# TheDatumOrg/VAQ

Hardware: AMD Instinct MI355X
Metric: queries/sec (ADC search, recall@100 reported alongside) (higher is better)
Workload: dtype f32; 1 GPU; sift1m-shaped d128 m8x256 nq10k k100; rows=1000000, rows_per_gpu=1000000, queries_per_gpu=10000, k=100, code_bytes=8, codes=encoded, method=HEAP/EA (exhaustive)

## Files before the change

### vaq_amd/csrc/vaq_kernels.h

```cpp
#ifndef VAQ_KERNELS_H_
#define VAQ_KERNELS_H_

#include <hip/hip_runtime.h>
#include <stdint.h>

#include "refine_owner.h"

namespace vaq {

struct SubDesc {
  int ncent;
  int bits;
  int bit_off;
  int lut_off;
  int cent_off;
  int word;
  int shift;
  int pad;
};

enum Layout { LAYOUT_BYTES = 0, LAYOUT_BITS = 1 };
enum EarlyAbandon { EA_NONE = 0, EA_QUEUE = 1, EA_INPLACE = 2 };

constexpr int TILE_ROWS = 64;
// ... 19 lines not shown
  int n_buckets;
  int bucket_shift;
  int bucket_t;
  int n_hot;
  unsigned long long *stats;
  int no_skip;
  const int *first_sub;
  const float *lut;
  int lut_floats;
  int lds_subs;
  int lut_lds_entries;
  int nq;
  int k;
  int kp;
  int ccap;
  int qcap;
  int q_cw_words;
  int nwaves;
  int ea;
  unsigned *g_thr;
  int qb;
  int n_slices;
  int64_t slice_rows;
  int64_t slice_stride;
  int share_thr;
  const int *slice_order;
  const int *qorder;
  int seq;
  int32_t *final_labels;
  float *final_dist;
  int64_t id_base;
  int *part_cnt;
  int bf_carry;
  int bf_pool;
  int defer_units, defer_mode, defer_cap;
  unsigned *defer_count;
  struct DeferRec *defer_list;
  unsigned *bm_done;
  int bf;
  int ti;
  const int *ti_order;
  const float *ti_qcc;
  const int *ti_nvisit;
  const float *ti_xcc;
  int ti_rowcap;
  int ti_cap;
  int sqrt_out;
  float *part_d;
  int *part_id;
};

hipError_t launch_project(const float *X, int64_t n, int D, const float *E, float *out,
                          hipStream_t st, int checked = 0);
hipError_t launch_lut_build(const float *qproj, int nq, int D, int M, int L,
                            const SubDesc *sub, const float *cent_t, int lut_floats, int max_ncent,
                            float *lut, hipStream_t st, int min_ncent = 1);
hipError_t launch_lut_expand(const float *lut_packed, int nq, int M, const SubDesc *sub,
                             int lut_floats, int ksub, float *lut_ref, hipStream_t st);
hipError_t launch_encode(const float *Xp, int64_t n, int D, int M, int L, const SubDesc *sub,
                         const float *cent, uint16_t *codes, hipStream_t st);
hipError_t lut_fit_columns(const float *d_Xp, int64_t n, int D, const int *bits, float *d_cent_out, float *d_q_out,
                           int *d_bad, float *phase_ms, hipStream_t st);
hipError_t launch_lut_encode(const float *Xp, int64_t n, int D, const SubDesc *h_sub, const SubDesc *d_sub,
                             const float *d_pm, const float *d_cent, uint16_t *codes, int n_cu, hipStream_t st);
hipError_t launch_refine(const float *Q, int nq, int D, const float *dataset, const float *rows,
                         const int32_t *labels_in, int R, int k, int32_t *labels, float *dist,
                         hipStream_t st);
struct RowsRef {
  const void *p;
  int elem;
};
inline RowsRef rows_at(RowsRef r, size_t elems) {
  return RowsRef{static_cast<const char *>(r.p) + elems * (size_t)r.elem, r.elem};
}
size_t refine_rows_max_dim();
hipError_t lut_fit_columns(RowsRef d_Xp, int64_t n, int D, const int *bits, float *d_cent_out, float *d_q_out,
                           int *d_bad, float *phase_ms, hipStream_t st);
hipError_t launch_project(RowsRef X, int64_t n, int D, const float *E, float *out, hipStream_t st, int checked = 0);
hipError_t launch_refine_rows(const float *Q, int nq, int D, RowsRef rows, int64_t N, int64_t id_base,
                              const int32_t *labels_in, int R, int k, int exact, int32_t *labels, float *dist,
                              hipStream_t st);
hipError_t launch_refine_dist(const float *Q, int nq, int D, RowsRef rows, int64_t n, int64_t lo_label,
                              const int32_t *labels_in, int R, float *plane, hipStream_t st);
hipError_t launch_refine_select(const int32_t *labels_in, int nq, const float *planes, size_t plane_stride,
                                const RefineBounds &bounds, int R, int k, int exact, int32_t *labels, float *dist,
                                hipStream_t st);
hipError_t launch_widen_rows_u8(const uint8_t *src, int64_t elems, float *dst, hipStream_t st);
constexpr int XS_TILE = 256;
constexpr int XS_MAX_QG = 1024;
constexpr int XS_MAX_K1 = 1025;
struct XsParams {
  int nq, D;
  int64_t N, id_base;
  int k, cap;
  int S, G, qg;
  int64_t split_rows;
  float *buf_d;
  int *buf_id;
  float *part_d;
  int *part_id;
};
int exhaust_list_cap(int k);
size_t exhaust_register_max_dim();
int exhaust_blocks_per_cu(int D, int elem);
hipError_t launch_exhaust_select(const XsParams &p, const float *Q, RowsRef rows, hipStream_t st);
hipError_t launch_exhaust_replay(const float *Q, int nq, int D, RowsRef rows, int64_t N, int64_t id_base, int k,
                                 const int *list, const unsigned *count, int32_t *labels, float *dist, hipStream_t st);
hipError_t launch_exhaust_replay_link(const float *Q, int nq, int D, RowsRef rows, int64_t N, int64_t id_base, int k,
                                      const int *list, const unsigned *count, const float *hin_v, const int *hin_i,
                                      float *hout_v, int *hout_i, int finish, int32_t *labels, float *dist,
                                      hipStream_t st);
hipError_t launch_exhaust_scatter(int nq, int k, const int *list, const unsigned *count, const float *src_v,
                                  const int *src_i, int32_t *labels, float *dist, hipStream_t st);
int64_t packed_words(int64_t rows, int M, int layout, int W);
hipError_t launch_pack_codes(const uint16_t *codes_u16, int64_t row_begin, int64_t row_end,
                             int64_t out_row_end, int M, int layout, int W, const SubDesc *sub,
                             const uint32_t *perm, uint32_t *out, hipStream_t st);
hipError_t sort_by_first_code(const uint16_t *d_codes, int64_t n, int M, int bits0, int shift, int bits1,
                              int t, uint32_t *d_perm, int *d_bucket_start, hipStream_t st, int fine = 0,
                              int *d_sub_start = nullptr);
hipError_t launch_merge_rows(const uint32_t *old_codes, const uint32_t *old_perm, const int *old_start,
                             const uint32_t *new_codes, const uint32_t *new_perm, const int *new_start, int K0,
                             int64_t n_old, int64_t n_total, int M, int layout, int W, uint32_t *out_codes,
                             uint32_t *out_perm, hipStream_t st);
hipError_t launch_slice_order(const float *lut, int lut_floats, int nq, int qb, const int *bstart,
                              int n_buckets, int bucket_shift, int64_t slice_rows, int n_slices,
                              int64_t n_rows, int *order, hipStream_t st);
hipError_t launch_cost_order(const float *lut, int lut_floats, int nq, int n0, int shift, unsigned long long *keys,
                             int *order, hipStream_t st);
hipError_t launch_query_order(const float *lut, int lut_floats, int nq, int n0, int off1, int n1, int *order,
                              hipStream_t st);
void scan_geometry(int layout, int M, int k, int ea, int *kp, int *ccap, int *qcap);
size_t scan_lds_bytes(int layout, int M, int lut_floats, int qb, int k, int ea, int nwaves,
                      int n_buckets, int bucket_shift, int bucket_t);
int scan_wg_step_rows(int layout, int M);
hipError_t launch_scan(const ScanParams &p, int *grid_out, hipStream_t st);
bool scan_bf_supported(int layout, int M, int qb, int ea, int n_buckets, int seq);
size_t scan_bf_lds_bytes(int layout, int M, int lut_entries, int pool, int nwaves, int n_buckets, int bf_carry);
void scan_bf_pool_range(int k, int *lo, int *hi);
size_t merge_scratch_elems(int n_lists, int nq, int k);
hipError_t launch_defer_merge(const unsigned *defer_count, int defer_cap, const DeferRec *defer_list, int n_lists, int k,
                              const float *part_d, const int *part_id, const int *part_cnt, int64_t id_base,
                              int32_t *labels, float *dist, hipStream_t st);
hipError_t launch_merge(const float *part_d, const int *part_id, const int *part_cnt, int n_lists,
                        int64_t list_stride, int64_t query_stride, int nq, int k,
                        int64_t id_base, int in_final, int32_t *labels, float *dist,
                        unsigned *thr_out, float *scratch_d, int *scratch_id, hipStream_t st);

constexpr int BM_HIST_BINS = 64;
constexpr int BM_XCDS = 8;
struct BmParams {
  const uint32_t *codes;
  const uint32_t *perm;
  const int *bucket_start;
  int n_buckets, bucket_t;
  const int *sub_start;
  int M;
  const float *lut;
  int lut_floats;
  int nq, k, qb;
  int nwaves;
  unsigned *g_thr;
  unsigned long long *thr64;
  int init64;
  unsigned *done_key;
  unsigned *done_next;
  unsigned *fresh;
  int limit;
  int retry;
  unsigned *mask;
  int *cnt;
  int *qoff;
  int *fill;
  int *qlist;
  unsigned short *qkey;
  int *border;
  int *ioff;
  unsigned *tickets;
  int cap;
  float *cand_d;
  int *cand_id;
  unsigned *cand_cnt;
// ... 96 lines not shown
```

### vaq_amd/csrc/vaq_kernels.hip

```cpp
#include "vaq_scan.h"
#include "vaq_scan_bf.h"
#include "vaqhip_dev.h"

#include <cstring>
#include <rocprim/device/device_radix_sort.hpp>

#include <float.h>
#include <limits.h>

namespace vaq {
template <typename T>
__global__ void project_kernel(const T *__restrict__ X, int D,
                               const float *__restrict__ E, float *__restrict__ out, int checked) {
  extern __shared__ float xs[];
  __shared__ int bad;
  const int64_t r = blockIdx.x;
  if (threadIdx.x == 0) bad = 0;
  for (int j = threadIdx.x; j < D; j += blockDim.x) xs[j] = (float)X[r * D + j];
  __syncthreads();
  if (!E) {
    for (int j = threadIdx.x; j < D; j += blockDim.x)
      if (!(fabsf(xs[j]) <= FLT_MAX)) bad = 1;
    __syncthreads();
    const bool zero = checked && bad;
// ... 125 lines not shown
                                 float *__restrict__ lut, int only_small) {
  extern __shared__ float qs[];
  const int q = blockIdx.x, s = blockIdx.y;
  const SubDesc sd = sub[s];
  if ((int)(blockIdx.z * blockDim.x) >= sd.ncent) return;
  if (only_small && sd.ncent >= 8) return;
  for (int j = threadIdx.x; j < L; j += blockDim.x) qs[j] = qproj[(size_t)q * D + (size_t)s * L + j];
  __syncthreads();
  float *out = lut + (size_t)q * lut_floats + sd.lut_off;
  const float *cs = cent_t + sd.cent_off;
  const int K = sd.ncent;
#define Y(j) cs[(size_t)(j) * K + c]
  for (int c = blockIdx.z * blockDim.x + threadIdx.x; c < K; c += gridDim.z * blockDim.x) {
    float r;
    if (K >= 8) {
      float acc = 0.0f;
      for (int j = 0; j < L; j++) {
        float diff = qs[j] - Y(j);
        acc = __builtin_fmaf(diff, diff, acc);
      }
      r = acc;
    } else if (L == 1) {
      r = sqdiff(qs[0], Y(0));
    } else if (L == 2) {
      r = sqdiff(qs[0], Y(0)) + sqdiff(qs[1], Y(1));
    } else if (L == 4) {
      r = (sqdiff(qs[0], Y(0)) + sqdiff(qs[1], Y(1))) + (sqdiff(qs[2], Y(2)) + sqdiff(qs[3], Y(3)));
    } else if (L == 8) {
      float a0 = sqdiff(qs[0], Y(0)) + sqdiff(qs[4], Y(4));
      float a1 = sqdiff(qs[1], Y(1)) + sqdiff(qs[5], Y(5));
      float a2 = sqdiff(qs[2], Y(2)) + sqdiff(qs[6], Y(6));
      float a3 = sqdiff(qs[3], Y(3)) + sqdiff(qs[7], Y(7));
      r = (a0 + a1) + (a2 + a3);
    } else if (L == 12) {
      float a0 = (sqdiff(qs[0], Y(0)) + sqdiff(qs[4], Y(4))) + sqdiff(qs[8], Y(8));
      float a1 = (sqdiff(qs[1], Y(1)) + sqdiff(qs[5], Y(5))) + sqdiff(qs[9], Y(9));
      float a2 = (sqdiff(qs[2], Y(2)) + sqdiff(qs[6], Y(6))) + sqdiff(qs[10], Y(10));
      float a3 = (sqdiff(qs[3], Y(3)) + sqdiff(qs[7], Y(7))) + sqdiff(qs[11], Y(11));
      r = (a0 + a1) + (a2 + a3);
    } else {
      float res = 0.0f;
      for (int j = 0; j < L; j++) {
        float t = qs[j] - Y(j);
        res += t * t;
      }
      r = res;
    }
    out[c] = r;
  }
#undef Y
}

constexpr int LUT_QT = 8;
__global__ __launch_bounds__(256) void lut_build_batch_kernel(const float *__restrict__ qproj, int nq, int D, int L,
                                                              const SubDesc *__restrict__ sub,
                                                              const float *__restrict__ cent_t, int lut_floats,
                                                              float *__restrict__ lut) {
  extern __shared__ float qs[];
  const int q0 = blockIdx.x * LUT_QT, s = blockIdx.y;
  const SubDesc sd = sub[s];
  const int K = sd.ncent;
  if (K < 8) return;
  for (int i = threadIdx.x; i < LUT_QT * L; i += blockDim.x) {
    const int qt = i / L, j = i - qt * L;
    qs[i] = q0 + qt < nq ? qproj[(size_t)(q0 + qt) * D + (size_t)s * L + j] : 0.0f;
  }
  __syncthreads();
  const float *cs = cent_t + sd.cent_off;
  for (int c = threadIdx.x; c < K; c += blockDim.x) {
    float acc[LUT_QT];
#pragma unroll
    for (int qt = 0; qt < LUT_QT; qt++) acc[qt] = 0.0f;
    for (int j = 0; j < L; j++) {
      const float y = cs[(size_t)j * K + c];
#pragma unroll
      for (int qt = 0; qt < LUT_QT; qt++) {
        const float diff = qs[qt * L + j] - y;
        acc[qt] = __builtin_fmaf(diff, diff, acc[qt]);
      }
    }
#pragma unroll
    for (int qt = 0; qt < LUT_QT; qt++)
      if (q0 + qt < nq) lut[(size_t)(q0 + qt) * lut_floats + sd.lut_off + c] = acc[qt];
  }
}

hipError_t launch_lut_build(const float *qproj, int nq, int D, int M, int L, const SubDesc *sub,
                            const float *cent_t, int lut_floats, int max_ncent, float *lut,
                            hipStream_t st, int min_ncent) {
  if (nq == 0) return hipSuccess;
  (void)max_ncent;
  if (nq >= 2 * LUT_QT && max_ncent >= 8) {
    hipLaunchKernelGGL(lut_build_batch_kernel, dim3((nq + LUT_QT - 1) / LUT_QT, M), dim3(256),
                       LUT_QT * L * sizeof(float), st, qproj, nq, D, L, sub, cent_t, lut_floats, lut);
    hipError_t e = hipGetLastError();
    if (e != hipSuccess || min_ncent >= 8) return e;
    hipLaunchKernelGGL(lut_build_kernel, dim3(nq, M, 1), dim3(64), L * sizeof(float), st, qproj, D, L, sub, cent_t,
                       lut_floats, lut, 1);
    return hipGetLastError();
  }
  hipLaunchKernelGGL(lut_build_kernel, dim3(nq, M, 1), dim3(256), L * sizeof(float), st, qproj, D, L,
                     sub, cent_t, lut_floats, lut, 0);
  return hipGetLastError();
}

__global__ void lut_expand_kernel(const float *__restrict__ lp, int M,
                                  const SubDesc *__restrict__ sub, int lut_floats, int ksub,
                                  float *__restrict__ lr) {
  const int q = blockIdx.x, s = blockIdx.y;
  const SubDesc sd = sub[s];
  for (int c = threadIdx.x; c < ksub; c += blockDim.x)
    lr[((size_t)q * M + s) * ksub + c] =
        c < sd.ncent ? lp[(size_t)q * lut_floats + sd.lut_off + c] : 0.0f;
}

hipError_t launch_lut_expand(const float *lut_packed, int nq, int M, const SubDesc *sub,
                             int lut_floats, int ksub, float *lut_ref, hipStream_t st) {
  if (nq == 0) return hipSuccess;
  hipLaunchKernelGGL(lut_expand_kernel, dim3(nq, M), dim3(256), 0, st, lut_packed, M, sub,
                     lut_floats, ksub, lut_ref);
  return hipGetLastError();
}

__global__ void pack_codes_kernel(const uint16_t *__restrict__ in, int64_t row_begin,
                                  int64_t row_end, int M, int layout, int W,
                                  const SubDesc *__restrict__ sub, const uint32_t *__restrict__ perm,
                                  uint32_t *__restrict__ out, int64_t t_begin, int64_t t_end) {
  const int64_t t = t_begin + (int64_t)blockIdx.x * blockDim.x + threadIdx.x;
  if (t >= t_end) return;
  uint32_t v = 0;
  if (layout == LAYOUT_BYTES) {
    const int wpr = M / 4;
    const int64_t r = t / wpr;
    const int w = (int)(t - r * wpr);
    if (r >= row_begin && r < row_end) {
      const uint16_t *c = in + ((perm ? (int64_t)perm[r] : r) - row_begin) * M + w * 4;
      v = (uint32_t)(c[0] & 0xff) | ((uint32_t)(c[1] & 0xff) << 8) |
          ((uint32_t)(c[2] & 0xff) << 16) | ((uint32_t)(c[3] & 0xff) << 24);
    }
  } else {
    const int64_t tile = t / ((int64_t)TILE_ROWS * W);
    const int rem = (int)(t - tile * TILE_ROWS * W);
    const int w = rem / TILE_ROWS;
    const int64_t r = tile * TILE_ROWS + (rem % TILE_ROWS);
    if (r >= row_begin && r < row_end) {
      const int64_t src = (perm ? (int64_t)perm[r] : r) - row_begin;
      for (int s = 0; s < M; s++) {
// ... 278 lines not shown
  for (int q = wave; q < P; q += nwaves) {
    unsigned long long key = ~0ull;
    if (q < nq) {
      const float *l = lut + (size_t)q * lut_floats;
      unsigned a[2];
#pragma unroll
      for (int t = 0; t < 2; t++) {
        const int off = t == 0 ? 0 : off1, n = t == 0 ? n0 : n1;
        unsigned long long best = ~0ull;
        for (int e = lane; e < n; e += 64) {
          const float x = l[off + e];
          const unsigned long long c = ((unsigned long long)(x == x ? float_to_bits(x) : 0xffffffffu) << 32) | (unsigned)e;
          best = c < best ? c : best;
        }
#pragma unroll
        for (int o = 32; o > 0; o >>= 1) {
          const unsigned long long x = __shfl_xor(best, o);
          best = x < best ? x : best;
        }
        a[t] = (unsigned)(best & 0xffffu);
      }
      key = ((unsigned long long)((a[0] << 16) | a[1]) << 32) | (unsigned)q;
    }
    if (lane == 0) qk[q] = key;
  }
  __syncthreads();
  for (int size = 2; size <= P; size <<= 1)
    for (int stride = size >> 1; stride > 0; stride >>= 1) {
      for (int t = tid; t < (P >> 1); t += QORDER_THREADS) {
        const int i = 2 * t - (t & (stride - 1));
        const int j = i + stride;
        const unsigned long long x = qk[i], y = qk[j];
        if ((x > y) == ((i & size) == 0)) { qk[i] = y; qk[j] = x; }
      }
      __syncthreads();
    }
  for (int i = tid; i < nq; i += QORDER_THREADS) order[i] = (int)(qk[i] & 0xffffffffu);
}

hipError_t launch_query_order(const float *lut, int lut_floats, int nq, int n0, int off1, int n1, int *order,
                              hipStream_t st) {
  if (nq <= 0 || nq > QORDER_MAX) return hipErrorInvalidValue;
  int P = 2;
  while (P < nq) P <<= 1;
  const size_t lds = (size_t)P * sizeof(unsigned long long);
  hipError_t e = hipFuncSetAttribute(reinterpret_cast<const void *>(query_order_kernel),
                                     hipFuncAttributeMaxDynamicSharedMemorySize, (int)lds);
  if (e != hipSuccess) return e;
  hipLaunchKernelGGL(query_order_kernel, dim3(1), dim3(QORDER_THREADS), lds, st, lut, lut_floats, nq, n0, off1, n1, order);
  return hipGetLastError();
}

template <int NREG>
__global__ __launch_bounds__(256) void query_cost_kernel(const float *__restrict__ lut, int lut_floats, int nq, int n0,
                                                         int shift, unsigned long long *__restrict__ keys) {
  const int lane = threadIdx.x & 63;
  const int q = blockIdx.x * 4 + (threadIdx.x >> 6);
  if (q >= nq) return;
  const float *l = lut + (size_t)q * lut_floats;
  const int nb_all = n0 >> shift;
  const int stride = nb_all > 64 * NREG ? nb_all / (64 * NREG) : 1;
  const int nb = nb_all / stride;
  unsigned v[NREG];
  unsigned vmin = 0xffffffffu, vmax = 0u;
#pragma unroll
  for (int i = 0; i < NREG; i++) {
    const int b = i * 64 + lane;
    unsigned m = 0xffffffffu;
    if (b < nb) {
      const int g = (16 >> shift) > 0 ? (16 >> shift) : 1;
      const int bb = (b / g) * g * stride + (b % g);
      for (int c = bb << shift; c < ((bb + 1) << shift); c++) {
        const float x = l[c];
        const unsigned xb = x == x ? float_to_bits(x) : 0xffffffffu;
        m = xb < m ? xb : m;
      }
    }
    v[i] = m;
    vmin = m < vmin ? m : vmin;
    vmax = (m != 0xffffffffu && m > vmax) ? m : vmax;
  }
#pragma unroll
  for (int o = 32; o > 0; o >>= 1) {
    const unsigned x = (unsigned)__shfl_xor((int)vmin, o), y = (unsigned)__shfl_xor((int)vmax, o);
    vmin = x < vmin ? x : vmin;
    vmax = y > vmax ? y : vmax;
  }
  int J = 16 / stride;
  J = J < 2 ? 2 : J;
  J = nb < J ? nb : J;
  unsigned lo = vmin, hi = vmax;
  if (lo > hi) lo = hi;
  while (lo < hi) {
    const unsigned mid = lo + ((hi - lo) >> 1);
    int c = 0;
#pragma unroll
    for (int i = 0; i < NREG; i++) c += __popcll(__ballot(v[i] <= mid));
    if (c >= J) hi = mid;
    else lo = mid + 1u;
  }
  float part = 0.0f;
  int below = 0;
#pragma unroll
  for (int i = 0; i < NREG; i++) {
    const bool lt = v[i] < lo;
    part += lt ? bits_to_float(v[i]) : 0.0f;
    below += __popcll(__ballot(lt));
  }
#pragma unroll
  for (int o = 32; o > 0; o >>= 1) part += __shfl_xor(part, o);
  const float v0 = bits_to_float(vmin < 0x7f800000u ? vmin : 0x7f800000u);
  const float spread = (part + (float)(J - below) * bits_to_float(lo)) - (float)J * v0;
  const unsigned kb = (spread == spread && spread >= 0.0f) ? float_to_bits(spread) : (spread < 0.0f ? 0u : 0x7f800000u);
  if (lane == 0) keys[q] = ((unsigned long long)kb << 32) | (unsigned)q;
}

constexpr int COST_CLASSES = 4096;
__global__ __launch_bounds__(QORDER_THREADS) void cost_sort_kernel(const unsigned long long *__restrict__ keys, int nq,
                                                                   int *__restrict__ order) {
  __shared__ unsigned hist[COST_CLASSES];
  __shared__ unsigned wave_tot[QORDER_THREADS / 64];
  const int tid = threadIdx.x, lane = tid & 63, wave = tid >> 6;
  for (int i = tid; i < COST_CLASSES; i += QORDER_THREADS) hist[i] = 0u;
  __syncthreads();
  for (int i = tid; i < nq; i += QORDER_THREADS) atomicAdd(&hist[(unsigned)(keys[i] >> 51) & (COST_CLASSES - 1)], 1u);
  __syncthreads();
  constexpr int PER = COST_CLASSES / QORDER_THREADS;
  unsigned c[PER], sum = 0u;
#pragma unroll
  for (int j = 0; j < PER; j++) {
    c[j] = hist[tid * PER + j];
    sum += c[j];
  }
  unsigned inc = sum;
#pragma unroll
  for (int o = 1; o < 64; o <<= 1) {
    const unsigned x = (unsigned)__shfl_up((int)inc, o);
    if (lane >= o) inc += x;
  }
  if (lane == 63) wave_tot[wave] = inc;
  __syncthreads();
  unsigned base = inc - sum;
  for (int w = 0; w < wave; w++) base += wave_tot[w];
#pragma unroll
  for (int j = 0; j < PER; j++) {
    hist[tid * PER + j] = base;
    base += c[j];
  }
  __syncthreads();
  for (int i = tid; i < nq; i += QORDER_THREADS) {
    const unsigned long long kq = keys[i];
    const unsigned pos = atomicAdd(&hist[(unsigned)(kq >> 51) & (COST_CLASSES - 1)], 1u);
    order[pos] = (int)(kq & 0xffffffffu);
  }
}

hipError_t launch_cost_order(const float *lut, int lut_floats, int nq, int n0, int shift, unsigned long long *keys,
                             int *order, hipStream_t st) {
  if (nq <= 0 || nq > QORDER_MAX || (n0 >> shift) > 1024 || (n0 >> shift) < 1) return hipErrorInvalidValue;
  hipLaunchKernelGGL(query_cost_kernel<4>, dim3((nq + 3) / 4), dim3(256), 0, st, lut, lut_floats, nq, n0, shift, keys);
  hipError_t e = hipGetLastError();
  if (e != hipSuccess) return e;
  hipLaunchKernelGGL(cost_sort_kernel, dim3(1), dim3(QORDER_THREADS), 0, st, keys, nq, order);
  return hipGetLastError();
}

static int rows_per_item(int layout, int M) { return (layout == LAYOUT_BYTES && M < 16) ? 16 / M : 1; }

int scan_wg_step_rows(int layout, int M) { return SCAN_MAX_THREADS * rows_per_item(layout, M); }

static int queue_code_words(int layout, int M, int ea) {
  return (layout == LAYOUT_BYTES && M <= 16 && ea == EA_QUEUE) ? M / 4 - 1 : 0;
}

void scan_geometry(int layout, int M, int k, int ea, int *kp, int *ccap, int *qcap) {
  int p2 = 1;
  while (p2 < k) p2 <<= 1;
  *kp = p2;
  *ccap = VAQ_CCAP;
  *qcap = ea == EA_QUEUE ? 128 : 0;
}

size_t scan_lds_bytes(int layout, int M, int lut_floats, int qb, int k, int ea, int nwaves,
                      int n_buckets, int bucket_shift, int bucket_t) {
  int kp, ccap, qcap;
  scan_geometry(layout, M, k, ea, &kp, &ccap, &qcap);
  size_t lut = (size_t)(layout == LAYOUT_BYTES ? M * 256 : lut_floats) * 4 * qb;
  lut = (lut + 15) & ~(size_t)15;
  const size_t sb = ((size_t)SEL_HDR_WORDS * 4 + (size_t)(kp + ccap) * 8 + 15) & ~(size_t)15;
  const size_t lbb = (bucket_shift > 0 || bucket_t > 0) ? (((size_t)n_buckets * 4 * qb + 15) & ~(size_t)15) : 0;
  return lut + (size_t)qb * sb + lbb + hot_bytes(n_buckets) +
         (size_t)nwaves * qcap * 4 * (1 + qb + queue_code_words(layout, M, ea));
}

size_t scan_ti_lds_bytes(int n_clusters) { return ti_lds_bytes(n_clusters); }

hipError_t launch_scan(const ScanParams &p_in, int *grid_out, hipStream_t st) {
  ScanParams p = p_in;
  p.q_cw_words = queue_code_words(p.layout, p.M, p.ea);
  const int nqb = (p.nq + p.qb - 1) / p.qb;
  const int total = nqb * p.n_slices;
  const int grid = ((total + 7) / 8) * 8;
  if (grid_out) *grid_out = grid;
  if (total == 0) return hipSuccess;
  if (p.bf) return launch_scan_bf(p, grid, st);
  size_t lds = scan_lds_bytes(p.layout, p.M, p.lut_lds_entries, p.qb, p.k, p.ea, p.nwaves, p.n_buckets,
                              p.bucket_shift, p.bucket_t);
  if (p.bucket_t < 0 || p.bucket_t > GMIN_MAX_BITS || (p.bucket_t > 0 && p.bucket_shift != 0))
    return hipErrorInvalidValue;
  if (p.ti) {
    if (p.qb != 1 || p.ea != EA_QUEUE || p.bucket_shift != 0 || p.bucket_t != 0 || p.n_hot != 0 || !p.sqrt_out)
      return hipErrorInvalidValue;
    if (p.ti_cap < 1 || p.ti_cap > p.n_buckets) return hipErrorInvalidValue;
    lds += ti_lds_bytes(p.ti_cap);
  } else if (p.sqrt_out) {
    return hipErrorInvalidValue;
  }
// ... 286 lines not shown
```

### vaq_amd/csrc/vaqhip_search.cpp

```cpp
#include "vaqhip_index.h"

using namespace vaqhost;

int vaqhost::check_search_args(const vaqhip_index *ix, const float *d_queries, int nq, int k, const int32_t *d_labels,
                               const float *d_dist, const char *method_err) {
  if (ix->N < 0) return fail(VAQHIP_ESTATE, "search before codes were set");
  if (ix->staged.open)
    return fail(VAQHIP_ESTATE, "a staged search is open on this index: call vaqhip_search_finish_device first");
  if (method_err) return fail(VAQHIP_ESTATE, "%s", method_err);
  if (nq < 0 || k <= 0) return fail(VAQHIP_EINVAL, "nq=%d k=%d", nq, k);
  if (k > VAQHIP_MAX_K) return fail(VAQHIP_EUNSUPPORTED, "k=%d > %d", k, VAQHIP_MAX_K);
  if (nq > 0 && (!d_queries || !d_labels || !d_dist)) return fail(VAQHIP_EINVAL, "null pointer");
  return VAQHIP_OK;
}

namespace {
int report_bm_debug(vaqhip_index *ix, const vaq::BmParams &bp, const int *limits, int r, const BmRoundInfo &bi,
                    hipStream_t st) {
  const int chunk = bi.chunk, n = bi.n;
  std::vector<unsigned> hq((size_t)3 * chunk);
  std::vector<int> hcnt((size_t)ix->n_buckets);
  HIP_TRY(hipStreamSynchronize(st));
  HIP_TRY(hipMemcpy(hq.data(), ix->w_bm_query.p, hq.size() * 4, hipMemcpyDeviceToHost));
  HIP_TRY(hipMemcpy(hcnt.data(), bp.cnt, hcnt.size() * 4, hipMemcpyDeviceToHost));
// ... 197 lines not shown
               "buckets tested %.1f visited %.1f | cycles total %.0f setup %.0f stepload-wait %.0f admit %.0f "
               "(fold %.0f lock-wait %.0f) drain %.0f | best-first: bootstrap %.0f round prep %.0f final (wave 0) %.0f setup up to the tables %.0f\n",
               h[0] / w, h[1] / w, h[2] / w, h[3] / w, h[4] / w, h[5] / w, h[9] / w, h[10] / w, h[6] / w, h[11] / w,
               h[12] / w, h[7] / w, h[13] / w, h[14] / w, h[8] / w, h[15] / w, h[16] / w, (double)h[17] / grid, h[18] / w);
  return VAQHIP_OK;
}
#endif

int group_queries(vaqhip_index *ix, const Plan &pl, int n, vaq::ScanParams &sp, hipStream_t st) {
  if (!(ix->ti_T == 0 && pl.qb > 1 && ix->M > 1 && n <= 16384 && !pl.ordered &&
        (ix->opt_group == 2 ||
         (ix->opt_group == 1 && n >= 4 * pl.qb && (double)ix->N * ((ix->total_bits + 7) / 8) > 256e6))))
    return VAQHIP_OK;
  HIP_TRY(ix->w_qorder.ensure((size_t)n * sizeof(int)));
  HIP_TRY(vaq::launch_query_order(ix->w_lut.as<float>(), ix->lut_floats, n, ix->sub[0].ncent, ix->sub[1].lut_off,
                                  ix->sub[1].ncent, ix->w_qorder.as<int>(), st));
  sp.qorder = ix->w_qorder.as<int>();
  return VAQHIP_OK;
}

int scan_chunk_ti(vaqhip_index *ix, const Plan &pl, const float *qp, int n, int k, vaq::ScanParams sp, int32_t *labels,
                  float *dist, hipEvent_t *ev, int *grid, hipStream_t st) {
  const int T = ix->ti_T;
  const int max_visit = ix->ti_visit < 1.0f ? (int)((float)T * ix->ti_visit) : T;
  HIP_TRY(vaq::launch_ti_plan(qp, n, ix->D, ix->ti_seg * ix->L, ix->d_ti_clusters_t.as<float>(), T,
                              ix->d_bstart.as<int>(), max_visit, k, ix->w_ti_order.as<int>(),
                              ix->w_ti_qcc.as<float>(), ix->w_ti_nvisit.as<int>(), st));
  if (ev) HIP_TRY(hipEventRecord(ev[3], st));
  sp.ti = 1;
  sp.ti_order = ix->w_ti_order.as<int>();
  sp.ti_qcc = ix->w_ti_qcc.as<float>();
  sp.ti_nvisit = ix->w_ti_nvisit.as<int>();
  sp.ti_xcc = ix->d_ti_xcc.as<float>();
  sp.ti_rowcap = (ix->methods & VAQHIP_METHOD_EA) ? 0x7fffffff : k;
  sp.ti_cap = pl.ti_cap;
  sp.sqrt_out = 1;
  sp.n_slices = pl.n_slices;
  sp.share_thr = pl.n_slices > 1;
  const bool direct = pl.n_slices == 1 && ix->N > 0;
  if (direct) {
    sp.final_labels = labels;
    sp.final_dist = dist;
  }
  if (ix->N > 0) HIP_TRY(vaq::launch_scan(sp, grid, st));
  if (ev) HIP_TRY(hipEventRecord(ev[4], st));
  if (!direct)
    HIP_TRY(vaq::launch_merge(sp.part_d, sp.part_id, nullptr, ix->N > 0 ? pl.n_slices : 0, k,
                              (int64_t)pl.n_slices * k, n, k, ix->id_base, 0, labels, dist, nullptr,
                              ix->w_ms_d.as<float>(), ix->w_ms_id.as<int>(), st));
  if (ev) HIP_TRY(hipEventRecord(ev[5], st));
  return VAQHIP_OK;
}

int seed_prepass(vaqhip_index *ix, const Plan &pl, int n, int k, vaq::ScanParams &sp, hipStream_t st) {
  if (ix->N > 0 && pl.seed_slices > 0) {
    sp.n_slices = pl.seed_slices;
    sp.slice_rows = pl.seed_rows;
    sp.slice_stride = pl.seed_stride;
    sp.share_thr = 1;
    sp.nwaves = 4;
    HIP_TRY(vaq::launch_scan(sp, nullptr, st));
    sp.nwaves = pl.nwaves;
    HIP_TRY(vaq::launch_merge(sp.part_d, sp.part_id, nullptr, pl.seed_slices, k, (int64_t)pl.seed_slices * k, n,
                              k, 0, 0, nullptr, nullptr, ix->w_thr.as<unsigned>(),
                              ix->w_ms_d.as<float>(), ix->w_ms_id.as<int>(), st));
  }
  if (pl.bf && pl.cost_order && pl.n_slices == 1 && ix->N > 0 && n >= COST_ORDER_MIN_QUERIES) {
    HIP_TRY(vaq::launch_cost_order(ix->w_lut.as<float>(), ix->lut_floats, n, ix->sub[0].ncent, ix->bucket_shift,
                                   ix->w_cost.as<unsigned long long>(), ix->w_qorder.as<int>(), st));
    sp.qorder = ix->w_qorder.as<int>();
  }
  return VAQHIP_OK;
}

int full_scan_params(vaqhip_index *ix, const Plan &pl, int n, vaq::ScanParams &sp, int32_t *labels, float *dist,
                     hipStream_t st) {
  sp.n_slices = pl.n_slices;
  sp.slice_rows = pl.slice_rows;
  sp.slice_stride = pl.slice_rows;
  sp.share_thr = pl.n_slices > 1;
  if (pl.ordered && ix->N > 0) {
    const int nqb = (n + pl.qb - 1) / pl.qb;
    HIP_TRY(ix->w_order.ensure((size_t)nqb * pl.n_slices * sizeof(int)));
    HIP_TRY(vaq::launch_slice_order(ix->w_lut.as<float>(), ix->lut_floats, n, pl.qb, ix->d_bstart.as<int>(),
                                    ix->n_buckets, ix->bucket_shift, pl.slice_rows, pl.n_slices, ix->N,
                                    ix->w_order.as<int>(), st));
    sp.slice_order = ix->w_order.as<int>();
  }
  if (pl.n_slices == 1 && ix->N > 0) {
    sp.final_labels = labels;
    sp.final_dist = dist;
  }
  sp.n_hot = (ix->opt_hot && sp.n_buckets >= 16 && sp.n_buckets <= 4096 &&
              (int64_t)sp.n_buckets <= (int64_t)(ix->layout == vaq::LAYOUT_BYTES ? ix->M * 256 : pl.lut_lds_entries) * pl.qb &&
              pl.slice_rows >= 8 * (ix->N / sp.n_buckets + 1)) ? ix->opt_hot : 0;
  sp.bf = pl.bf ? 1 : 0;
  sp.bf_carry = pl.bf_carry;
  sp.bf_pool = pl.bf_pool;
  return VAQHIP_OK;
}

vaq::BmParams bm_params(const vaqhip_index *ix, const Plan &pl, const vaq::ScanParams &sp, int chunk, int n, int k,
                        int32_t *labels, float *dist) {
  unsigned *qw = ix->w_bm_query.as<unsigned>();
  vaq::BmParams bp = {};
  bp.codes = sp.codes;
  bp.perm = sp.perm;
  bp.bucket_start = sp.bucket_start;
  bp.n_buckets = sp.n_buckets;
  bp.bucket_t = sp.bucket_t;
  bp.sub_start = (ix->sub_fine > 0 && ix->sub_fine + ix->bucket_t == 8 && ix->opt_bm_sub) ? ix->d_substart.as<int>() : nullptr;
  bp.M = ix->M;
  bp.lut = sp.lut;
  bp.lut_floats = sp.lut_floats;
  bp.nq = n;
  bp.k = k;
  bp.qb = pl.bm_qb;
  bp.nwaves = pl.bm_nwaves;
  bp.g_thr = sp.g_thr;
  bp.thr64 = ix->w_bm_thr64.as<unsigned long long>();
  bp.done_key = qw;
  bp.cand_cnt = qw + (size_t)chunk;
// ... 84 lines not shown
  tm.queries_per_pass = pl.qb;
  tm.slices = pl.n_slices;
  tm.workgroups = grid;
  tm.passes = (n + pl.qb - 1) / pl.qb;
  tm.lds_bytes = (int)pl.lds;
}

int search_core(vaqhip_index *ix, const float *d_queries, int nq, int k, int projected,
                int32_t *d_labels, float *d_dist, hipStream_t st, int32_t *stage_thr_out = nullptr) {
  const char *method_err = nullptr;
  if (((ix->methods & VAQHIP_METHOD_TI) != 0) != (ix->ti_T > 0))
    method_err = ix->ti_T > 0 ? "the rows are grouped by TI cluster: the method must include TI"
                              : "method TI needs vaqhip_index_set_ti_clusters first";
  if (int rc = check_search_args(ix, d_queries, nq, k, d_labels, d_dist, method_err)) return rc;
  if (nq == 0) return VAQHIP_OK;
  WS_SCOPE(ws, ix, st);
  bool timing = ix->opt_timing != 0;
  hipEvent_t *ev = nullptr;
  if (timing) {
    if (int rc = ensure_events(ix)) return rc;
    if (ix->ev_used >= vaqhip_index::EV_SETS) timing = false;
    else ev = ix->ev.data() + (size_t)ix->ev_used * 6;
  }
  vaqhip_timing tm = {};
  tm.deferred_queries = -1;
  Plan pl;
  const bool ti = ix->ti_T > 0;
  const int chunk = std::min(nq, QUERY_CHUNK);
  if (int rc = ti ? make_ti_plan(ix, chunk, k, &pl) : make_plan(ix, chunk, k, &pl)) return rc;
  if (stage_thr_out) {
    if (!(pl.bm && pl.bf && pl.n_slices == 1 && ix->N > 0 && nq <= QUERY_CHUNK && !ti))
      return fail(VAQHIP_EUNSUPPORTED, "a staged search needs the bucket-major rounds (streamed byte codes, >= 8 queries, "
                                       "at most %d per call)", QUERY_CHUNK);
    timing = false;
  }
  const bool do_project = !projected && (ix->has_eig || ix->seq);
  if (int rc = ensure_scan_workspaces(ix, pl, chunk, k, do_project)) return rc;
  if (timing && nq > chunk)
    return fail(VAQHIP_EUNSUPPORTED, "timing supports at most %d queries per call", QUERY_CHUNK);

  for (int q0 = 0; q0 < nq; q0 += chunk) {
    const int n = std::min(chunk, nq - q0);
    const float *dq = d_queries + (size_t)q0 * ix->D;
    const float *qp = dq;
    int32_t *labels = d_labels + (size_t)q0 * k;
    float *dist = d_dist + (size_t)q0 * k;
    if (timing) HIP_TRY(hipEventRecord(ev[0], st));
    if (do_project) {
      HIP_TRY(vaq::launch_project(dq, n, ix->D, ix->has_eig ? ix->d_eig.as<float>() : nullptr, ix->w_qproj.as<float>(), st,
                                  ix->seq ? 1 : 0));
      qp = ix->w_qproj.as<float>();
    }
    if (timing) HIP_TRY(hipEventRecord(ev[1], st));
    HIP_TRY(vaq::launch_lut_build(qp, n, ix->D, ix->M, ix->L, ix->d_sub.as<vaq::SubDesc>(),
                                  ix->d_cent_t.as<float>(), ix->lut_floats, 1 << ix->max_bits, ix->w_lut.as<float>(), st,
                                  1 << ix->min_bits));
    if (timing) HIP_TRY(hipEventRecord(ev[2], st));
    vaq::ScanParams sp = base_scan_params(ix, pl, n, k);
#if defined(VAQ_STATS) || defined(VAQ_PHASES)
    if (int rc = attach_stats(sp, st)) return rc;
#endif
    int grid = 0;
    if (int rc = group_queries(ix, pl, n, sp, st)) return rc;
    if (pl.n_slices > 1 || pl.seed_slices > 0 || pl.bm)
      HIP_TRY(hipMemsetD32Async(reinterpret_cast<hipDeviceptr_t>(ix->w_thr.p), 0x7f7fffff, n, st));
    if (ti) {
      if (int rc = scan_chunk_ti(ix, pl, qp, n, k, sp, labels, dist, timing ? ev : nullptr, &grid, st)) return rc;
      fill_timing_ti(tm, pl, n, grid);
      continue;
    }
    if (int rc = seed_prepass(ix, pl, n, k, sp, st)) return rc;
    if (timing) HIP_TRY(hipEventRecord(ev[3], st));
    if (int rc = full_scan_params(ix, pl, n, sp, labels, dist, st)) return rc;
    const bool direct = pl.n_slices == 1 && ix->N > 0;
    const bool bm = pl.bm && pl.bf && direct;
    const bool defer = pl.bf && pl.defer_units > 0 && direct && !bm;
    vaq::BmParams bp = {};
    if (bm || defer)
      if (int rc = cap_first_pass(ix, pl, bm, chunk, n, k, labels, dist, sp, bp, st)) return rc;
    if (bm && pl.bm_boot) {
      HIP_TRY(vaq::launch_bm_boot(bp, ix->N, st));
    } else if (ix->N > 0) {
      HIP_TRY(vaq::launch_scan(sp, &grid, st));
    }
    if (bm) {
      const BmRoundInfo bi = {chunk, n, pl.bm_cap, pl.bm_qb, pl.defer_units};
      if (int rc = run_bucket_major(ix, bp, sp, bi, pl.bm_boot, k, stage_thr_out, d_labels, d_dist, st)) return rc;
      if (stage_thr_out) {
        ix->last = tm;
        return ws.finish();
      }
    }
    if (defer || bm)
      if (int rc = bm_fallback(ix, sp, sp.defer_cap, k, labels, dist, st)) return rc;
#ifdef VAQ_PHASES
    if (pl.bf)
      if (int rc = report_phases(sp, st)) return rc;
#endif
#ifdef VAQ_STATS
    if (int rc = report_stats(sp, grid, st)) return rc;
#endif
    if (timing) HIP_TRY(hipEventRecord(ev[4], st));
    if (!direct)
      HIP_TRY(vaq::launch_merge(sp.part_d, sp.part_id, (pl.seed_slices > 0 || pl.ordered) ? sp.part_cnt : nullptr,
                                ix->N > 0 ? pl.n_slices : 0, k, (int64_t)pl.n_slices * k, n, k, ix->id_base, 0, labels,
                                dist, nullptr, ix->w_ms_d.as<float>(), ix->w_ms_id.as<int>(), st));
    if (timing) HIP_TRY(hipEventRecord(ev[5], st));
    fill_timing(tm, pl, n, grid, bm, defer);
  }
// ... 285 lines not shown
```

Before: 21.31 million queries/s.

## Fuse query cost-key computation into LUT build and parallelize cost scatter

The first subquantizer's LUT-build blocks now also compute each query's cost key, staging the tile in LDS, so the separate query_cost_kernel pass over the LUT is skipped. The single-block histogram sort is replaced by a multi-block scatter kernel: each block recomputes the class histogram with packed 16-bit prefix counts so it can place its own queries without a global sync. This removes one kernel launch and a LUT re-read and spreads the scatter across many workgroups. The cost is redundant per-block histogramming and extra LDS and work in the LUT build.

After: 21.63 million queries/s, median of 6. 1.5% higher.

```diff
diff --git a/vaq_amd/csrc/vaq_kernels.h b/vaq_amd/csrc/vaq_kernels.h
--- a/vaq_amd/csrc/vaq_kernels.h
+++ b/vaq_amd/csrc/vaq_kernels.h
@@ -95,9 +95,13 @@
 
 hipError_t launch_project(const float *X, int64_t n, int D, const float *E, float *out,
                           hipStream_t st, int checked = 0);
+struct CostKeys {
+  unsigned long long *keys;
+  int n0, shift;
+};
 hipError_t launch_lut_build(const float *qproj, int nq, int D, int M, int L,
                             const SubDesc *sub, const float *cent_t, int lut_floats, int max_ncent,
-                            float *lut, hipStream_t st, int min_ncent = 1);
+                            float *lut, hipStream_t st, int min_ncent = 1, const CostKeys *ck = nullptr);
 hipError_t launch_lut_expand(const float *lut_packed, int nq, int M, const SubDesc *sub,
                              int lut_floats, int ksub, float *lut_ref, hipStream_t st);
 hipError_t launch_encode(const float *Xp, int64_t n, int D, int M, int L, const SubDesc *sub,
@@ -171,6 +175,7 @@
                               int64_t n_rows, int *order, hipStream_t st);
 hipError_t launch_cost_order(const float *lut, int lut_floats, int nq, int n0, int shift, unsigned long long *keys,
                              int *order, hipStream_t st);
+hipError_t launch_cost_scatter(const unsigned long long *keys, int nq, int *order, hipStream_t st);
 hipError_t launch_query_order(const float *lut, int lut_floats, int nq, int n0, int off1, int n1, int *order,
                               hipStream_t st);
 void scan_geometry(int layout, int M, int k, int ea, int *kp, int *ccap, int *qcap);
diff --git a/vaq_amd/csrc/vaq_kernels.hip b/vaq_amd/csrc/vaq_kernels.hip
--- a/vaq_amd/csrc/vaq_kernels.hip
+++ b/vaq_amd/csrc/vaq_kernels.hip
@@ -201,10 +201,16 @@
 }
 
 constexpr int LUT_QT = 8;
+constexpr int COST_KEY_LDS_ENTRIES = 256;
+template <int NREG>
+__device__ __forceinline__ unsigned cost_key_bits(const float *l, int n0, int shift, int lane);
+__device__ __forceinline__ void cost_key_emit(unsigned kb, int q, unsigned long long *__restrict__ keys);
+
 __global__ __launch_bounds__(256) void lut_build_batch_kernel(const float *__restrict__ qproj, int nq, int D, int L,
                                                               const SubDesc *__restrict__ sub,
                                                               const float *__restrict__ cent_t, int lut_floats,
-                                                              float *__restrict__ lut) {
+                                                              float *__restrict__ lut,
+                                                              unsigned long long *__restrict__ keys, int shift) {
   extern __shared__ float qs[];
   const int q0 = blockIdx.x * LUT_QT, s = blockIdx.y;
   const SubDesc sd = sub[s];
@@ -215,6 +221,9 @@
     qs[i] = q0 + qt < nq ? qproj[(size_t)(q0 + qt) * D + (size_t)s * L + j] : 0.0f;
   }
   __syncthreads();
+  const bool rank = keys != nullptr && s == 0;
+  const bool rank_lds = rank && K <= COST_KEY_LDS_ENTRIES;
+  float *t0 = qs + LUT_QT * L;
   const float *cs = cent_t + sd.cent_off;
   for (int c = threadIdx.x; c < K; c += blockDim.x) {
     float acc[LUT_QT];
@@ -229,19 +238,36 @@
       }
     }
 #pragma unroll
-    for (int qt = 0; qt < LUT_QT; qt++)
+    for (int qt = 0; qt < LUT_QT; qt++) {
       if (q0 + qt < nq) lut[(size_t)(q0 + qt) * lut_floats + sd.lut_off + c] = acc[qt];
-  }
-}
+      if (rank_lds) t0[qt * K + c] = acc[qt];
+    }
+  }
+  if (!rank) return;
+  __threadfence_block();
+  __syncthreads();
+  const int lane = threadIdx.x & 63;
+  for (int qt = threadIdx.x >> 6; qt < LUT_QT && q0 + qt < nq; qt += blockDim.x >> 6) {
+    const int q = q0 + qt;
+    const unsigned kb = rank_lds ? cost_key_bits<4>(t0 + qt * K, K, shift, lane)
+                                 : cost_key_bits<4>(lut + (size_t)q * lut_floats + sd.lut_off, K, shift, lane);
+    if (lane == 0) cost_key_emit(kb, q, keys);
+  }
+}
+
+static bool cost_order_shape_ok(int nq, int n0, int shift);
 
 hipError_t launch_lut_build(const float *qproj, int nq, int D, int M, int L, const SubDesc *sub,
                             const float *cent_t, int lut_floats, int max_ncent, float *lut,
-                            hipStream_t st, int min_ncent) {
+                            hipStream_t st, int min_ncent, const CostKeys *ck) {
   if (nq == 0) return hipSuccess;
   (void)max_ncent;
+  if (ck && !(nq >= 2 * LUT_QT && ck->n0 >= 8 && cost_order_shape_ok(nq, ck->n0, ck->shift))) return hipErrorInvalidValue;
   if (nq >= 2 * LUT_QT && max_ncent >= 8) {
-    hipLaunchKernelGGL(lut_build_batch_kernel, dim3((nq + LUT_QT - 1) / LUT_QT, M), dim3(256),
-                       LUT_QT * L * sizeof(float), st, qproj, nq, D, L, sub, cent_t, lut_floats, lut);
+    size_t lds = LUT_QT * L * sizeof(float);
+    if (ck && ck->n0 <= COST_KEY_LDS_ENTRIES) lds += (size_t)LUT_QT * ck->n0 * sizeof(float);
+    hipLaunchKernelGGL(lut_build_batch_kernel, dim3((nq + LUT_QT - 1) / LUT_QT, M), dim3(256), lds, st, qproj, nq, D, L,
+                       sub, cent_t, lut_floats, lut, ck ? ck->keys : nullptr, ck ? ck->shift : 0);
     hipError_t e = hipGetLastError();
     if (e != hipSuccess || min_ncent >= 8) return e;
     hipLaunchKernelGGL(lut_build_kernel, dim3(nq, M, 1), dim3(64), L * sizeof(float), st, qproj, D, L, sub, cent_t,
@@ -626,12 +652,7 @@
 }
 
 template <int NREG>
-__global__ __launch_bounds__(256) void query_cost_kernel(const float *__restrict__ lut, int lut_floats, int nq, int n0,
-                                                         int shift, unsigned long long *__restrict__ keys) {
-  const int lane = threadIdx.x & 63;
-  const int q = blockIdx.x * 4 + (threadIdx.x >> 6);
-  if (q >= nq) return;
-  const float *l = lut + (size_t)q * lut_floats;
+__device__ __forceinline__ unsigned cost_key_bits(const float *l, int n0, int shift, int lane) {
   const int nb_all = n0 >> shift;
   const int stride = nb_all > 64 * NREG ? nb_all / (64 * NREG) : 1;
   const int nb = nb_all / stride;
@@ -685,26 +706,44 @@
   for (int o = 32; o > 0; o >>= 1) part += __shfl_xor(part, o);
   const float v0 = bits_to_float(vmin < 0x7f800000u ? vmin : 0x7f800000u);
   const float spread = (part + (float)(J - below) * bits_to_float(lo)) - (float)J * v0;
-  const unsigned kb = (spread == spread && spread >= 0.0f) ? float_to_bits(spread) : (spread < 0.0f ? 0u : 0x7f800000u);
-  if (lane == 0) keys[q] = ((unsigned long long)kb << 32) | (unsigned)q;
+  return (spread == spread && spread >= 0.0f) ? float_to_bits(spread) : (spread < 0.0f ? 0u : 0x7f800000u);
 }
 
 constexpr int COST_CLASSES = 4096;
-__global__ __launch_bounds__(QORDER_THREADS) void cost_sort_kernel(const unsigned long long *__restrict__ keys, int nq,
-                                                                   int *__restrict__ order) {
-  __shared__ unsigned hist[COST_CLASSES];
+
+__device__ __forceinline__ unsigned cost_class(unsigned long long key) { return (unsigned)(key >> 51) & (COST_CLASSES - 1); }
+
+__device__ __forceinline__ void cost_key_emit(unsigned kb, int q, unsigned long long *__restrict__ keys) {
+  keys[q] = ((unsigned long long)kb << 32) | (unsigned)q;
+}
+
+template <int NREG>
+__global__ __launch_bounds__(256) void query_cost_kernel(const float *__restrict__ lut, int lut_floats, int nq, int n0,
+                                                         int shift, unsigned long long *__restrict__ keys) {
+  const int lane = threadIdx.x & 63;
+  const int q = blockIdx.x * 4 + (threadIdx.x >> 6);
+  if (q >= nq) return;
+  const unsigned kb = cost_key_bits<NREG>(lut + (size_t)q * lut_floats, n0, shift, lane);
+  if (lane == 0) cost_key_emit(kb, q, keys);
+}
+
+static_assert(QORDER_MAX < (1 << 16), "a class's two counts share one word");
+__global__ __launch_bounds__(QORDER_THREADS) void cost_scatter_kernel(const unsigned long long *__restrict__ keys, int nq,
+                                                                      int *__restrict__ order) {
+  __shared__ unsigned cnt[COST_CLASSES];
   __shared__ unsigned wave_tot[QORDER_THREADS / 64];
   const int tid = threadIdx.x, lane = tid & 63, wave = tid >> 6;
-  for (int i = tid; i < COST_CLASSES; i += QORDER_THREADS) hist[i] = 0u;
-  __syncthreads();
-  for (int i = tid; i < nq; i += QORDER_THREADS) atomicAdd(&hist[(unsigned)(keys[i] >> 51) & (COST_CLASSES - 1)], 1u);
+  const int mine0 = blockIdx.x * QORDER_THREADS;
+  for (int i = tid; i < COST_CLASSES; i += QORDER_THREADS) cnt[i] = 0u;
+  __syncthreads();
+  for (int i = tid; i < nq; i += QORDER_THREADS) atomicAdd(&cnt[cost_class(keys[i])], i < mine0 ? 0x10001u : 1u);
   __syncthreads();
   constexpr int PER = COST_CLASSES / QORDER_THREADS;
   unsigned c[PER], sum = 0u;
 #pragma unroll
   for (int j = 0; j < PER; j++) {
-    c[j] = hist[tid * PER + j];
-    sum += c[j];
+    c[j] = cnt[tid * PER + j];
+    sum += c[j] & 0xffffu;
   }
   unsigned inc = sum;
 #pragma unroll
@@ -718,25 +757,35 @@
   for (int w = 0; w < wave; w++) base += wave_tot[w];
 #pragma unroll
   for (int j = 0; j < PER; j++) {
-    hist[tid * PER + j] = base;
-    base += c[j];
-  }
-  __syncthreads();
-  for (int i = tid; i < nq; i += QORDER_THREADS) {
-    const unsigned long long kq = keys[i];
-    const unsigned pos = atomicAdd(&hist[(unsigned)(kq >> 51) & (COST_CLASSES - 1)], 1u);
-    order[pos] = (int)(kq & 0xffffffffu);
-  }
+    cnt[tid * PER + j] = base + (c[j] >> 16);
+    base += c[j] & 0xffffu;
+  }
+  __syncthreads();
+  const int i = mine0 + tid;
+  if (i >= nq) return;
+  const unsigned long long kq = keys[i];
+  const unsigned pos = atomicAdd(&cnt[cost_class(kq)], 1u);
+  if (pos < (unsigned)nq) order[pos] = (int)(kq & 0xffffffffu);
+}
+
+static bool cost_order_shape_ok(int nq, int n0, int shift) {
+  return nq > 0 && nq <= QORDER_MAX && (n0 >> shift) <= 1024 && (n0 >> shift) >= 1;
+}
+
+hipError_t launch_cost_scatter(const unsigned long long *keys, int nq, int *order, hipStream_t st) {
+  if (nq <= 0 || nq > QORDER_MAX) return hipErrorInvalidValue;
+  hipLaunchKernelGGL(cost_scatter_kernel, dim3((nq + QORDER_THREADS - 1) / QORDER_THREADS), dim3(QORDER_THREADS), 0, st,
+                     keys, nq, order);
+  return hipGetLastError();
 }
 
 hipError_t launch_cost_order(const float *lut, int lut_floats, int nq, int n0, int shift, unsigned long long *keys,
                              int *order, hipStream_t st) {
-  if (nq <= 0 || nq > QORDER_MAX || (n0 >> shift) > 1024 || (n0 >> shift) < 1) return hipErrorInvalidValue;
+  if (!cost_order_shape_ok(nq, n0, shift)) return hipErrorInvalidValue;
   hipLaunchKernelGGL(query_cost_kernel<4>, dim3((nq + 3) / 4), dim3(256), 0, st, lut, lut_floats, nq, n0, shift, keys);
   hipError_t e = hipGetLastError();
   if (e != hipSuccess) return e;
-  hipLaunchKernelGGL(cost_sort_kernel, dim3(1), dim3(QORDER_THREADS), 0, st, keys, nq, order);
-  return hipGetLastError();
+  return launch_cost_scatter(keys, nq, order, st);
 }
 
 static int rows_per_item(int layout, int M) { return (layout == LAYOUT_BYTES && M < 16) ? 16 / M : 1; }
diff --git a/vaq_amd/csrc/vaqhip_search.cpp b/vaq_amd/csrc/vaqhip_search.cpp
--- a/vaq_amd/csrc/vaqhip_search.cpp
+++ b/vaq_amd/csrc/vaqhip_search.cpp
@@ -273,6 +273,13 @@
   return VAQHIP_OK;
 }
 
+bool ranks_queries(const vaqhip_index *ix, const Plan &pl, int n) {
+  return pl.bf && pl.cost_order && pl.n_slices == 1 && ix->N > 0 && n >= COST_ORDER_MIN_QUERIES;
+}
+bool keys_from_table_build(const vaqhip_index *ix, const Plan &pl, int n) {
+  return ranks_queries(ix, pl, n) && ix->sub[0].ncent >= 8;
+}
+
 int seed_prepass(vaqhip_index *ix, const Plan &pl, int n, int k, vaq::ScanParams &sp, hipStream_t st) {
   if (ix->N > 0 && pl.seed_slices > 0) {
     sp.n_slices = pl.seed_slices;
@@ -286,9 +293,12 @@
                               k, 0, 0, nullptr, nullptr, ix->w_thr.as<unsigned>(),
                               ix->w_ms_d.as<float>(), ix->w_ms_id.as<int>(), st));
   }
-  if (pl.bf && pl.cost_order && pl.n_slices == 1 && ix->N > 0 && n >= COST_ORDER_MIN_QUERIES) {
-    HIP_TRY(vaq::launch_cost_order(ix->w_lut.as<float>(), ix->lut_floats, n, ix->sub[0].ncent, ix->bucket_shift,
-                                   ix->w_cost.as<unsigned long long>(), ix->w_qorder.as<int>(), st));
+  if (ranks_queries(ix, pl, n)) {
+    if (keys_from_table_build(ix, pl, n))
+      HIP_TRY(vaq::launch_cost_scatter(ix->w_cost.as<unsigned long long>(), n, ix->w_qorder.as<int>(), st));
+    else
+      HIP_TRY(vaq::launch_cost_order(ix->w_lut.as<float>(), ix->lut_floats, n, ix->sub[0].ncent, ix->bucket_shift,
+                                     ix->w_cost.as<unsigned long long>(), ix->w_qorder.as<int>(), st));
     sp.qorder = ix->w_qorder.as<int>();
   }
   return VAQHIP_OK;
@@ -479,9 +489,10 @@
       qp = ix->w_qproj.as<float>();
     }
     if (timing) HIP_TRY(hipEventRecord(ev[1], st));
+    const vaq::CostKeys ck = {ix->w_cost.as<unsigned long long>(), ix->sub[0].ncent, ix->bucket_shift};
     HIP_TRY(vaq::launch_lut_build(qp, n, ix->D, ix->M, ix->L, ix->d_sub.as<vaq::SubDesc>(),
                                   ix->d_cent_t.as<float>(), ix->lut_floats, 1 << ix->max_bits, ix->w_lut.as<float>(), st,
-                                  1 << ix->min_bits));
+                                  1 << ix->min_bits, !ti && keys_from_table_build(ix, pl, n) ? &ck : nullptr));
     if (timing) HIP_TRY(hipEventRecord(ev[2], st));
     vaq::ScanParams sp = base_scan_params(ix, pl, n, k);
 #if defined(VAQ_STATS) || defined(VAQ_PHASES)
```
